# LeeBY68/Hier-SLAM

Measured on AMD Instinct MI355X. Metric: fwd+bwd renders/sec @1200x680, 500k Gaussians, 4-level tree; grad max-abs-err vs ref, higher is better.
Workload: dtype f32; 1 GPU; semantic fwd+bwd render, 1200x680, P=500000 slam Gaussians, K=26 semantic channels, dense upstream grads on colour/semantic/depth/median/opacity; P=500000, visible=480888, num_rendered=1136056, width=1200, height=680, K=26, parallelism=single GPU, keyframes_per_rank=1

## Files before the change

### hier-slam_amd/csrc/hsr_api.hip

```cpp
#include <stdarg.h>

#include <chrono>
#include <time.h>
#include <stdio.h>
#include <stdlib.h>
#include <string.h>

#include <mutex>
#include <type_traits>
#include <vector>

#include "../../include/hsr_rasterizer.h"
#include "hsr_tile_common.h"

namespace {

thread_local char g_err[512] = "";

template <typename T>
inline void take(char*& p, T*& out, size_t count)
{
    uintptr_t a = (reinterpret_cast<uintptr_t>(p) + 255) & ~(uintptr_t)255;
    out = reinterpret_cast<T*>(a);
    p = reinterpret_cast<char*>(out + count);
// ... 134 lines not shown
    if (d < 0 || d >= HSR_MAX_DEVICES) {
        hsr_set_error("device index %d out of range", d);
        return HSR_ERR_INVALID_ARGUMENT;
    }
    g_pc = &g_counters_by_device[d];
    if (!g_pinned) {
        HSR_HIP_CHECK(hipHostMalloc(reinterpret_cast<void**>(&g_pinned), 64, hipHostMallocPortable | hipHostMallocMapped));
        g_pinned[0] = g_pinned[1] = g_pinned[2] = 0;
        HSR_HIP_CHECK(hipHostGetDevicePointer(reinterpret_cast<void**>(&g_pinned_dev), g_pinned, 0));
    }
    return HSR_OK;
}
int read_counter_begin(const uint32_t* dev, hipStream_t stream)
{
    int rc;
    if ((rc = counter_buffer()) != HSR_OK) return rc;
    if (!g_counter_event) HSR_HIP_CHECK(hipEventCreateWithFlags(&g_counter_event, hipEventDisableTiming));
    HSR_HIP_CHECK(hipMemcpyAsync(g_pinned, dev, sizeof(uint32_t), hipMemcpyDeviceToHost, stream));
    HSR_HIP_CHECK(hipMemcpyAsync(g_pinned + 2, dev + 1, sizeof(uint32_t), hipMemcpyDeviceToHost, stream));
    HSR_HIP_CHECK(hipEventRecord(g_counter_event, stream));
    return HSR_OK;
}
thread_local double g_host_wait_ms = 0.0;
thread_local int g_last_per_tile = 0;
int read_counter_end(uint32_t* host_out)
{
    const auto t0 = std::chrono::steady_clock::now();
    HSR_HIP_CHECK(hipEventSynchronize(g_counter_event));
    g_host_wait_ms += std::chrono::duration<double, std::milli>(std::chrono::steady_clock::now() - t0).count();
    *host_out = g_pinned[0];
    return HSR_OK;
}
int poll_counter(uint32_t seq, hipStream_t stream, uint32_t* host_out, volatile uint32_t* slot = nullptr)
{
    const auto t0 = std::chrono::steady_clock::now();
    if (slot) {
        unsigned spins = 0;
        uint32_t cur;
        while ((cur = __atomic_load_n(&slot[1], __ATOMIC_ACQUIRE)) != seq) {
            if (cur != 0 && (int32_t)(cur - seq) > 0) {
                hsr_set_error("non-blocking forward: this call's num_rendered was overwritten — more than %d non-blocking forwards were "
                              "started on the device before it was resolved (resolve or drop earlier ones first)", HSR_ASYNC_SLOTS - 1);
                return HSR_ERR_INVALID_ARGUMENT;
            }
            if ((++spins & 0xFFFu) == 0) {
                const double el = std::chrono::duration<double>(std::chrono::steady_clock::now() - t0).count();
                if (el > 10.0) {
// ... 169 lines not shown
            seq = ++g_counter_seq;
            if (seq == 0) seq = ++g_counter_seq;
            slot_dev = g_pinned_dev;
        }
        StageTimer tm(HSR_STAGE_FWD_DUPLICATE, stream);
        hsr_launch_bin_count(plan, P, radii, tiles_x, tiles_y, g, bin_scratch, im.ranges, stream, slot_dev, seq);
    } else {
        StageTimer tm(HSR_STAGE_FWD_SCAN, stream);
        hsr_launch_scan_block_sums(P, g, stream);
    }
    HSR_LAUNCH_CHECK(in.debug, stream);

    if (!binned && (rc = read_counter_begin(g.counters, stream)) != HSR_OK) return rc;

    RenderFwdArgs ra;
    ra.W = W; ra.H = H; ra.K = in.semantic ? in.K : 0; ra.semantic = in.semantic;
    ra.ranges = im.ranges; ra.point_list = nullptr; ra.masks = nullptr; ra.means2D = g.means2D; ra.conic_opacity = g.conic_opacity;
    ra.depths = g.depths; ra.colors = in.colors_precomp ? in.colors_precomp : g.rgb; ra.semantics = in.semantics;
    ra.rec = g.rec;
    ra.final_T = im.final_T; ra.n_contrib = im.n_contrib; ra.median_pos = im.median_pos;
    ra.out_color = in.out_color; ra.out_semantic = in.out_semantic; ra.out_depth = in.out_depth;
    ra.out_median_depth = in.out_median; ra.out_opacity = in.out_opacity; ra.out_mask = in.out_mask;
    ra.bin = BinDevRef{nullptr, nullptr, 0};
    if (!in.semantic && !in.out_mask) {
        hsr_set_error("out_mask is NULL");
        return HSR_ERR_INVALID_ARGUMENT;
    }

    bool speculated = false;
    if (will_speculate) {
        const BinDevRef ref{static_cast<char*>(binning->ptr), reinterpret_cast<const uint32_t*>(g.counters), binning->capacity};
        BinState none{nullptr, nullptr, nullptr, nullptr, nullptr};
        {
            StageTimer tm(HSR_STAGE_FWD_DUPLICATE, stream);
            hsr_launch_bin_emit(plan, P, radii, tiles_x, tiles_y, g, bin_scratch, im.ranges, nullptr, stream, &ref);
        }
        {
            StageTimer tm(HSR_STAGE_FWD_SORT, stream);
            hsr_launch_tile_sort(none, T, P, im.ranges, stream, &ref, g_last_per_tile);
        }
        ra.bin = ref;
        {
            StageTimer tm(HSR_STAGE_FWD_RENDER, stream);
            hsr_launch_render_forward(ra, stream);
        }
        HSR_HIP_CHECK(hipGetLastError());
        speculated = true;
    }
    if (go_async) {
        ticket->seq = seq;
        ticket->device = slot_device;
        ticket->slot = slot_host;
        ticket->binning_base = static_cast<char*>(binning->ptr);
        ticket->binning_capacity = binning->capacity;
        ticket->prefiltered = in.prefiltered;
        return HSR_PENDING;
    }

    uint32_t R32 = 0;
    if ((rc = binned ? poll_counter(seq, stream, &R32) : read_counter_end(&R32)) != HSR_OK) return rc;
    if (R32 > 0x7fffffffu) {
        hsr_set_error("num_rendered %u overflows int", R32);
        return HSR_ERR_INVALID_ARGUMENT;
    }
    const int R = (int)R32;
    if (in.prefiltered && __atomic_load_n(&g_pinned[2], __ATOMIC_RELAXED) != 0) {
        hsr_set_error("Point is filtered although prefiltered is set. This shouldn't happen!");
        return HSR_ERR_INVALID_ARGUMENT;
    }
    if (speculated) {
        BinState chk;
        const BinDevRef ref{static_cast<char*>(binning->ptr), nullptr, binning->capacity};
        g_last_per_tile = R / (T > 0 ? T : 1);
        if (hsr_bin_resolve(ref, R32, &chk)) return R;
        hsr_launch_bin_count(plan, P, radii, tiles_x, tiles_y, g, bin_scratch, im.ranges, stream, g_pinned_dev, seq);
        ra.bin = BinDevRef{nullptr, nullptr, 0};
    }

    char* bptr;
    if ((rc = acquire(binning, hsr_required_binning_bytes(R), "binning", &bptr)) != HSR_OK) return rc;
    BinState b;
    hsr_carve_bin(bptr, R, &b);

    if (binned) {
        StageTimer tm(HSR_STAGE_FWD_DUPLICATE, stream);
        hsr_launch_bin_emit(plan, P, radii, tiles_x, tiles_y, g, bin_scratch, im.ranges, b.keys, stream);
    }
    if (binned) {
        HSR_LAUNCH_CHECK(in.debug, stream);
        StageTimer tm(HSR_STAGE_FWD_SORT, stream);
        if (R > 0) hsr_launch_tile_sort(b, T, P, im.ranges, stream, nullptr, R / (T > 0 ? T : 1));
    } else {
        const bool emit_sorted = hsr_sort_emit_into_sorted_buffers(end_bit);
        uint64_t* emit_k = emit_sorted ? b.keys : b.keys_unsorted;
        uint32_t* emit_v = emit_sorted ? b.vals : b.vals_unsorted;
        {
            StageTimer tm(HSR_STAGE_FWD_DUPLICATE, stream);
            BinState be = b;
            be.keys_unsorted = emit_k;
            be.vals_unsorted = emit_v;
            hsr_launch_duplicate(P, radii, tiles_x, tiles_y, g, be, im.ranges, stream);
        }
        HSR_LAUNCH_CHECK(in.debug, stream);
        StageTimer tm(HSR_STAGE_FWD_SORT, stream);
        if ((rc = hsr_launch_sort_pairs(b, R, end_bit, T, im.ranges, stream)) != HSR_OK) return rc;
    }
    HSR_LAUNCH_CHECK(in.debug, stream);

    ra.point_list = b.vals;
    ra.masks = b.vals_unsorted;
    {
        StageTimer tm(HSR_STAGE_FWD_RENDER, stream);
        hsr_launch_render_forward(ra, stream);
    }
// ... 480 lines not shown
```

### hier-slam_amd/csrc/hsr_common.h

```cpp
#pragma once
#include <hip/hip_runtime.h>
#include <stddef.h>
#include <stdint.h>

#define HSR_TILE_X 16
#define HSR_TILE_Y 16
#define HSR_TILE_PIX 256
#define HSR_NUM_CHANNELS 3

struct GeomState {
    float* depths;
    float2* means2D;
    float4* conic_opacity;
    float* cov3D;
    float* rgb;
    uint8_t* clamped;
    uint32_t* tiles_touched;
    uint32_t* point_offsets;
    int* radii;
    uint32_t* block_sums;
    uint32_t* counters;
    float4* rec;
};
struct ImgState {
// ... 70 lines not shown
    const float* projmatrix;
    const float* cam_pos;
    float tan_fovx, tan_fovy, focal_x, focal_y;
    int* radii;
    int prefiltered;
    int tiles_x, tiles_y;
};

int hsr_launch_mark_visible(int P, const float* means3D, const float* view, const float* proj, uint8_t* present,
                            hipStream_t stream);
int hsr_launch_preprocess(const PreprocessArgs& a, GeomState& g, hipStream_t stream);
int hsr_launch_scan_block_sums(int P, GeomState& g, hipStream_t stream);
int hsr_launch_duplicate(int P, const int* radii, int tiles_x, int tiles_y, GeomState& g, BinState& b, uint2* ranges,
                         hipStream_t stream);
int hsr_launch_sort_pairs(BinState& b, int R, int end_bit, int T, uint2* ranges, hipStream_t stream);
struct HsrBinPlan { int nblk, per_block; };
bool hsr_bin_plan(int P, int T, size_t scratch_words, HsrBinPlan* plan);
int hsr_launch_bin_count(const HsrBinPlan& plan, int P, const int* radii, int tiles_x, int tiles_y, GeomState& g, uint32_t* scratch,
                         uint2* ranges, hipStream_t stream, uint32_t* host_counter = nullptr, uint32_t host_seq = 0);
int hsr_launch_bin_emit(const HsrBinPlan& plan, int P, const int* radii, int tiles_x, int tiles_y, GeomState& g, const uint32_t* scratch,
                        uint2* ranges, uint64_t* comp, hipStream_t stream, const BinDevRef* ref = nullptr);
int hsr_launch_tile_sort(BinState& b, int T, int P, const uint2* ranges, hipStream_t stream, const BinDevRef* ref = nullptr,
                         int avg_per_tile_hint = 0);
int hsr_sort_tile_passes(int end_bit);
bool hsr_sort_emit_into_sorted_buffers(int end_bit);
int hsr_launch_tile_ranges(int R, int T, const uint64_t* keys, uint2* ranges, hipStream_t stream);
int hsr_launch_tile_ranges_only(int R, const uint64_t* keys, uint2* ranges, hipStream_t stream);

struct RenderFwdArgs {
    int W, H, K, semantic;
    const uint2* ranges;
    const uint32_t* point_list;
    uint32_t* masks;
    const float2* means2D;
    const float4* conic_opacity;
    const float* depths;
    const float* colors;
    const float4* rec;
    const float* semantics;
    float* final_T;
    uint32_t* n_contrib;
    uint32_t* median_pos;
    float* out_color;
    float* out_semantic;
    float* out_depth;
    float* out_median_depth;
    float* out_opacity;
    float* out_mask;
    BinDevRef bin;
};
int hsr_launch_render_forward(const RenderFwdArgs& a, hipStream_t stream);

struct RenderBwdArgs {
    int W, H, K, semantic, P;
    const float* bg;
    const uint2* ranges;
    const uint32_t* point_list;
    const uint32_t* masks;
    const float2* means2D;
    const float4* conic_opacity;
    const float* depths;
    const float* colors;
    const float4* rec;
    const float* final_T;
    const uint32_t* n_contrib;
    const uint32_t* median_pos;
    const float* dL_dpix;
    const float* dL_dpix_sem;
    const float* dL_dpix_depth;
    const float* dL_dpix_median;
    const float* dL_dpix_opacity;
    float* dL_dmean2D;
// ... 59 lines not shown
```

### hier-slam_amd/csrc/hsr_render_fwd.hip

```cpp

#include "hsr_tile_common.h"

#ifdef HSR_TRACE
__device__ unsigned long long g_hsr_trace_fwd[16384 * 8];
extern "C" int hsr_debug_read_trace_fwd(unsigned long long* host, int n)
{
    return (int)hipMemcpyFromSymbol(host, HIP_SYMBOL(g_hsr_trace_fwd), sizeof(unsigned long long) * (size_t)n);
}
#define TRF_NOW() clock64()
#define TRF_ADD(acc, t0) (acc) += (unsigned long long)(clock64() - (t0))
#else
#define TRF_NOW() 0ll
#define TRF_ADD(acc, t0) ((void)0)
#endif

namespace {

template <int W>
__device__ __forceinline__ void quad_fma_words(float (&s)[16], const float (&x)[4], float w)
{
    static_assert(W >= 1 && W <= 4, "1..4 words = 4..16 channels per block");
    if constexpr (W == 4) {
        asm("s_nop 1\n\t"
            "v_fmac_f32_dpp %0, %16, %20 quad_perm:[0,0,0,0] row_mask:0xf bank_mask:0xf\n\t"
// ... 33 lines not shown
    } else if constexpr (W == 2) {
        asm("s_nop 1\n\t"
            "v_fmac_f32_dpp %0, %8, %10 quad_perm:[0,0,0,0] row_mask:0xf bank_mask:0xf\n\t"
            "v_fmac_f32_dpp %1, %8, %10 quad_perm:[1,1,1,1] row_mask:0xf bank_mask:0xf\n\t"
            "v_fmac_f32_dpp %2, %8, %10 quad_perm:[2,2,2,2] row_mask:0xf bank_mask:0xf\n\t"
            "v_fmac_f32_dpp %3, %8, %10 quad_perm:[3,3,3,3] row_mask:0xf bank_mask:0xf\n\t"
            "v_fmac_f32_dpp %4, %9, %10 quad_perm:[0,0,0,0] row_mask:0xf bank_mask:0xf\n\t"
            "v_fmac_f32_dpp %5, %9, %10 quad_perm:[1,1,1,1] row_mask:0xf bank_mask:0xf\n\t"
            "v_fmac_f32_dpp %6, %9, %10 quad_perm:[2,2,2,2] row_mask:0xf bank_mask:0xf\n\t"
            "v_fmac_f32_dpp %7, %9, %10 quad_perm:[3,3,3,3] row_mask:0xf bank_mask:0xf"
            : "+v"(s[0]), "+v"(s[1]), "+v"(s[2]), "+v"(s[3]), "+v"(s[4]), "+v"(s[5]), "+v"(s[6]), "+v"(s[7])
            : "v"(x[0]), "v"(x[1]), "v"(w));
    } else {
        asm("s_nop 1\n\t"
            "v_fmac_f32_dpp %0, %4, %5 quad_perm:[0,0,0,0] row_mask:0xf bank_mask:0xf\n\t"
            "v_fmac_f32_dpp %1, %4, %5 quad_perm:[1,1,1,1] row_mask:0xf bank_mask:0xf\n\t"
            "v_fmac_f32_dpp %2, %4, %5 quad_perm:[2,2,2,2] row_mask:0xf bank_mask:0xf\n\t"
            "v_fmac_f32_dpp %3, %4, %5 quad_perm:[3,3,3,3] row_mask:0xf bank_mask:0xf"
            : "+v"(s[0]), "+v"(s[1]), "+v"(s[2]), "+v"(s[3])
            : "v"(x[0]), "v"(w));
    }
}

template <int KC, bool BASE, bool MASK, bool ALIGNED, bool PF = false>
__global__ void __launch_bounds__(256, KC <= 26 ? (KC == 16 ? 5 : 4) : (PF ? (KC <= 48 ? 4 : (KC <= 80 ? 3 : 2)) : 1)) render_fwd_kernel(RenderFwdArgs a, int c0)
{
    constexpr int BATCH = KC <= 32 ? (KC > 26 ? 200 : 240)
                                   : (KC <= 48 ? 152 : ((KC <= 64 || KC == 74) ? 144 : (KC <= 80 ? 136 : (KC <= 112 ? 144 : 128))));
    static_assert(KC <= 32 || PF, "batch sizes beyond 32 channels assume the touched rows (PF)");
    constexpr int RW = (KC + 2 + 3) & ~3;
    constexpr bool QS = PF && KC > 0;
    constexpr int NGF = QS ? RW / 16 : 0;
    constexpr int REM = QS ? (RW % 16) / 4 : 0;
    __shared__ float4 s_rec[BATCH * 2];
    __shared__ float4 s_row[BATCH * (RW / 4)];
    __shared__ uint8_t s_sublist[16 * HSR_SUB_LSTRIDE];
    __shared__ uint8_t s_subcnt[4][16];
    __shared__ int s_wdone[4];

    const int tile = hsr_block_tile(blockIdx.x, ((a.W + HSR_TILE_X - 1) / HSR_TILE_X) * ((a.H + HSR_TILE_Y - 1) / HSR_TILE_Y));
    if (tile >= ((a.W + HSR_TILE_X - 1) / HSR_TILE_X) * ((a.H + HSR_TILE_Y - 1) / HSR_TILE_Y)) return;
    const int t = threadIdx.x, wv = t >> 6;
    if (a.bin.base) {
        BinState bs;
        if (!hsr_bin_resolve(a.bin, *a.bin.R_dev, &bs)) {
            hsr_poison_tile(a, tile, t, BASE, c0, KC);
            return;
        }
        a.point_list = bs.vals;
        a.masks = bs.vals_unsorted;
    }
    const TileGeom tg = tile_geom_sub(tile, a.W, a.H, t);
    const bool inside = tg.inside;
    const size_t N = (size_t)a.W * a.H;
    float pfx = tg.pfx, pfy = tg.pfy;
    asm volatile("" : "+v"(pfx), "+v"(pfy));
    const float tile_x0 = (float)(tg.tx * HSR_TILE_X), tile_y0 = (float)(tg.ty * HSR_TILE_Y);

    unsigned long long tr_bar = 0, tr_stage = 0, tr_blend = 0, tr_iters = 0, tr_pub = 0;
    (void)tr_pub;
    const long long tr_t0 = TRF_NOW();
    long long tr_t1 = tr_t0;
    (void)tr_bar; (void)tr_stage; (void)tr_blend; (void)tr_iters; (void)tr_t0; (void)tr_t1;
    const uint2 range = a.ranges[tile];
    const int n = (int)(range.y - range.x);

    float T = 1.0f;
    uint32_t last_contributor = 0;
    float C0 = 0, C1 = 0, C2 = 0, Dd = 0, Mm = 0;
    uint32_t median_at = 0;
    float median_D = 15.0f;
    float S[KC > 0 ? KC : 1];
#pragma unroll
// ... 31 lines not shown
            if (KC > 0 && PF) {
                const float* row = a.semantics + id * (size_t)a.K + c0;
                const int last = min(KC, a.K - c0) - 1;
#pragma unroll
                for (int c = 0; c < NPF; c++) pf_t[c] = row[min(16 * c, last)];
            } else if (KC > 0) {
                if (ALIGNED) {
                    const float2* row = reinterpret_cast<const float2*>(a.semantics + id * (size_t)KC);
#pragma unroll
                    for (int q = 0; q < KC / 2; q++) {
                        const float2 v = row[q];
                        p_sem[PF ? 0 : 2 * q] = v.x;
                        p_sem[PF ? 0 : 2 * q + 1] = v.y;
                    }
                } else {
                    const float* row = a.semantics + id * (size_t)a.K + c0;
#pragma unroll
                    for (int c = 0; c < KC; c++) p_sem[PF ? 0 : c] = (c0 + c < a.K) ? row[c] : 0.f;
                }
            }
        }
    };
    if (n > 0) {
        const int id0 = fetch_id(0);
        id_next = fetch_id(BATCH);
        load_record(id0);
    }
    auto resolve_median = [&](int start) {
        if (BASE && median_at > (uint32_t)start) {
            const int j = (int)median_at - 1 - start;
            constexpr int c = KC + 1;
            constexpr int pos = (QS && c / 16 < NGF) ? (16 * (c / 16) + 4 * (c % 4) + (c % 16) / 4) : c;
            median_D = reinterpret_cast<const float*>(s_row)[j * RW + pos];
        }
    };


    for (int start = 0; start < n; start += BATCH) {
        const bool wave_done = __ballot(!done) == 0ull;
        if ((t & 63) == 0) s_wdone[wv] = wave_done;
        const long long tb0 = TRF_NOW();
        (void)tb0;
        __syncthreads();
        TRF_ADD(tr_bar, tb0);
        if (start == 0) tr_t1 = TRF_NOW();
        const long long ts0 = TRF_NOW();
        (void)ts0;
        if (s_wdone[0] & s_wdone[1] & s_wdone[2] & s_wdone[3]) break;
// ... 227 lines not shown
        }
        if (KC > 0) {
#pragma unroll
            for (int c = 0; c < KC; c++)
                if (c0 + c < a.K) a.out_semantic[(size_t)(c0 + c) * N + pix_id] = S[c];
        }
    }
#ifdef HSR_TRACE
    if ((t & 63) == 0) {
        const int wid = tile * 4 + wv;
        if (wid < 16384) {
            unsigned long long* o = g_hsr_trace_fwd + (size_t)wid * 8;
            o[0] = (unsigned long long)(clock64() - tr_t0);
            o[1] = (unsigned long long)(tr_t1 - tr_t0);
            o[2] = tr_bar; o[3] = tr_stage; o[4] = tr_blend;
            o[5] = (unsigned long long)(clock64() - tr_t2);
            o[6] = tr_iters;
            o[7] = tr_pub;
        }
    }
#endif
}

}

int hsr_launch_render_forward(const RenderFwdArgs& a, hipStream_t stream)
{
    const dim3 grid(hsr_tile_grid(((a.W + HSR_TILE_X - 1) / HSR_TILE_X) * ((a.H + HSR_TILE_Y - 1) / HSR_TILE_Y))), block(256);
    if (!a.semantic) {
        render_fwd_kernel<0, true, true, false><<<grid, block, 0, stream>>>(a, 0);
        return HSR_OK;
    }
    if (a.K >= 27 && a.K <= 128 && a.K != 74 && a.K != 102) {
        if (a.K <= 32) render_fwd_kernel<32, true, false, false, true><<<grid, block, 0, stream>>>(a, 0);
        else if (a.K <= 48) render_fwd_kernel<48, true, false, false, true><<<grid, block, 0, stream>>>(a, 0);
        else if (a.K <= 64) render_fwd_kernel<64, true, false, false, true><<<grid, block, 0, stream>>>(a, 0);
        else if (a.K <= 80) render_fwd_kernel<80, true, false, false, true><<<grid, block, 0, stream>>>(a, 0);
        else if (a.K <= 96) render_fwd_kernel<96, true, false, false, true><<<grid, block, 0, stream>>>(a, 0);
        else if (a.K <= 112) render_fwd_kernel<112, true, false, false, true><<<grid, block, 0, stream>>>(a, 0);
        else render_fwd_kernel<128, true, false, false, true><<<grid, block, 0, stream>>>(a, 0);
        return HSR_OK;
    }
    switch (a.K) {
    case 0: render_fwd_kernel<0, true, false, false><<<grid, block, 0, stream>>>(a, 0); return HSR_OK;
    case 16: render_fwd_kernel<16, true, false, true><<<grid, block, 0, stream>>>(a, 0); return HSR_OK;
    case 26: render_fwd_kernel<26, true, false, true><<<grid, block, 0, stream>>>(a, 0); return HSR_OK;
    case 74: render_fwd_kernel<74, true, false, true, true><<<grid, block, 0, stream>>>(a, 0); return HSR_OK;
    case 102: render_fwd_kernel<102, true, false, true, true><<<grid, block, 0, stream>>>(a, 0); return HSR_OK;
    default:
        render_fwd_kernel<32, true, false, false><<<grid, block, 0, stream>>>(a, 0);
        for (int c0 = 32; c0 < a.K; c0 += 32) render_fwd_kernel<32, false, false, false><<<grid, block, 0, stream>>>(a, c0);
        return HSR_OK;
    }
}
```

### hier-slam_amd/csrc/hsr_sort.hip

```cpp
#include "hsr_common.h"

namespace {

constexpr int SORT_THREADS = 256;
constexpr int SORT_ITEMS = 16;
constexpr int SORT_TILE = SORT_THREADS * SORT_ITEMS;
static_assert(SORT_TILE == HSR_SORT_TILE, "hsr_common.h sizes the histogram scratch");

__global__ void __launch_bounds__(SORT_THREADS) sort_hist_kernel(const uint64_t* __restrict__ keys, int n, int shift,
                                                                 uint32_t mask, int nblocks, uint32_t* __restrict__ hist)
{
    __shared__ uint32_t h[256];
    h[threadIdx.x] = 0;
    __syncthreads();
    const int base = blockIdx.x * SORT_TILE;
#pragma unroll 4
    for (int i = 0; i < SORT_ITEMS; i++) {
        const int j = base + i * SORT_THREADS + threadIdx.x;
        if (j < n) atomicAdd(&h[(uint32_t)(keys[j] >> shift) & mask], 1u);
    }
    __syncthreads();
    hist[(size_t)threadIdx.x * nblocks + blockIdx.x] = h[threadIdx.x];
}

// ... 86 lines not shown
        wcnt[0][threadIdx.x] = g;
        wcnt[1][threadIdx.x] = g + c0;
        wcnt[2][threadIdx.x] = g + c0 + c1;
        wcnt[3][threadIdx.x] = g + c0 + c1 + c2;
    }
    __syncthreads();
#pragma unroll
    for (int r = 0; r < SORT_ITEMS; r++) {
        const int j = base + r * 64 + lane;
        if (j < n) {
            const uint32_t d = (uint32_t)(key[r] >> shift) & mask;
            const uint32_t pos = wcnt[w][d] + rank[r];
            kout[pos] = key[r];
            vout[pos] = val[r];
        }
    }
}

}

uint32_t hsr_sort_hist_entries(int R) { return hsr_sort_hist_entries_inline((uint32_t)(R > 0 ? R : 0)); }


constexpr int TS_MAX = 2048;

__device__ __forceinline__ void ts_block_radix(uint64_t* ka, uint32_t* va, uint64_t* kb, uint32_t* vb, int r0, int n,
                                               uint32_t* hist , uint32_t (*wcnt)[256], int gid_passes)
{
    const int t = threadIdx.x, lane = t & 63, w = t >> 6;
    const uint64_t lt = (1ull << lane) - 1ull;
    const int npass = gid_passes + 4;
    for (int pass = 0; pass < npass; pass++) {
        const bool on_gid = pass < gid_passes;
        const int shift = 8 * (on_gid ? pass : pass - gid_passes);
        hist[t] = 0;
#pragma unroll
        for (int i = 0; i < 4; i++) wcnt[i][t] = 0;
        __syncthreads();
        for (int i = t; i < n; i += 256)
            atomicAdd(&hist[((on_gid ? va[r0 + i] : (uint32_t)ka[r0 + i]) >> shift) & 255u], 1u);
        __syncthreads();
        {
            const uint32_t v = hist[t];
            uint32_t inc = v;
#pragma unroll
            for (int o = 1; o < 64; o <<= 1) {
                const uint32_t x = __shfl_up(inc, o);
                if (lane >= o) inc += x;
            }
            __shared__ uint32_t wt[4];
            if (lane == 63) wt[w] = inc;
            __syncthreads();
            uint32_t off = 0;
#pragma unroll
            for (int i = 0; i < 4; i++) off += i < w ? wt[i] : 0u;
            hist[t] = off + inc - v;
        }
        __syncthreads();
        for (int c = 0; c < n; c += 256) {
            const int i = c + t;
            const bool valid = i < n;
            const uint64_t k = valid ? ka[r0 + i] : 0ull;
            const uint32_t v = valid ? va[r0 + i] : 0u;
            const uint32_t d = ((on_gid ? v : (uint32_t)k) >> shift) & 255u;
            uint64_t m = __ballot(valid);
#pragma unroll
            for (int b = 0; b < 8; b++) {
                const bool bit = (d >> b) & 1u;
                const uint64_t bal = __ballot(bit);
                m &= bit ? bal : ~bal;
            }
            const uint32_t before = __popcll(m & lt);
            if (valid && before == 0) wcnt[w][d] = (uint32_t)__popcll(m);
            __syncthreads();
            if (valid) {
                uint32_t pos = hist[d] + before;
#pragma unroll
                for (int i2 = 0; i2 < 4; i2++) pos += i2 < w ? wcnt[i2][d] : 0u;
                kb[r0 + pos] = k;
                vb[r0 + pos] = v;
            }
            __syncthreads();
            hist[t] += wcnt[0][t] + wcnt[1][t] + wcnt[2][t] + wcnt[3][t];
#pragma unroll
            for (int i2 = 0; i2 < 4; i2++) wcnt[i2][t] = 0;
            __syncthreads();
        }
        uint64_t* tk = ka; ka = kb; kb = tk;
        uint32_t* tv = va; va = vb; vb = tv;
        __threadfence_block();
    }
    if (npass & 1) {
        __syncthreads();
        for (int i = t; i < n; i += 256) {
            kb[r0 + i] = ka[r0 + i];
            vb[r0 + i] = va[r0 + i];
        }
    }
}

constexpr int TP_MAX = 1024;
constexpr int TQ_MAX = 2048;

template <int E, int NT>
__device__ __forceinline__ void net_bitonic(uint64_t (&x)[E], int tid, ulonglong2* buf)
{
    constexpr int N = NT * E;
#pragma unroll
    for (int k = 2; k <= N; k <<= 1) {
#pragma unroll
        for (int j = k >> 1; j > 0; j >>= 1) {
            if (j < E) {
#pragma unroll
                for (int r = 0; r < E; r++) {
                    if ((r & j) == 0) {
                        const bool up = k < E ? ((r & k) == 0) : (((E * tid) & k) == 0);
                        const uint64_t a = x[r], b = x[r + j];
                        const bool sw = (a > b) == up;
                        x[r] = sw ? b : a;
                        x[r + j] = sw ? a : b;
                    }
                }
            } else {
                const int m = j / E;
                const bool cross = m >= 64;
#pragma unroll
                for (int q = 0; q < E / 2; q++) buf[q * NT + tid] = make_ulonglong2(x[2 * q], x[2 * q + 1]);
                if (cross) {
                    __syncthreads();
                } else {
                    __builtin_amdgcn_fence(__ATOMIC_RELEASE, "wavefront");
                    __builtin_amdgcn_wave_barrier();
                    __builtin_amdgcn_fence(__ATOMIC_ACQUIRE, "wavefront");
                }
                const bool keep_min = ((tid & m) == 0) == (((E * tid) & k) == 0);
#pragma unroll
                for (int q = 0; q < E / 2; q++) {
                    const ulonglong2 y = buf[q * NT + (tid ^ m)];
                    const uint64_t a0 = x[2 * q], a1 = x[2 * q + 1];
                    x[2 * q] = keep_min ? (a0 < y.x ? a0 : y.x) : (a0 > y.x ? a0 : y.x);
                    x[2 * q + 1] = keep_min ? (a1 < y.y ? a1 : y.y) : (a1 > y.y ? a1 : y.y);
                }
                if (cross) {
                    __syncthreads();
                } else {
                    __builtin_amdgcn_fence(__ATOMIC_RELEASE, "wavefront");
                    __builtin_amdgcn_wave_barrier();
                    __builtin_amdgcn_fence(__ATOMIC_ACQUIRE, "wavefront");
                }
            }
        }
    }
}

__device__ __forceinline__ void block_sort_tile(int tile, const uint2* __restrict__ ranges, uint64_t* __restrict__ keys,
                                                uint32_t* __restrict__ vals, uint64_t* __restrict__ keys_alt,
                                                uint32_t* __restrict__ vals_alt, int gid_passes, int composite_in, uint64_t* comp,
                                                uint32_t* hist, uint32_t (*wcnt)[256])
{
    const uint2 rg = ranges[tile];
    const int r0 = (int)rg.x, n = (int)(rg.y - rg.x);
    const int t = threadIdx.x;
    const uint64_t my_tile_hi = (uint64_t)tile << 32;
    if (n <= 0) return;
    if (n == 1 || n > TS_MAX) {
        if (composite_in) {
            for (int i = t; i < n; i += 256) {
                const uint64_t c = keys[r0 + i];
                keys[r0 + i] = my_tile_hi | (c >> 32);
                vals[r0 + i] = (uint32_t)c;
            }
            __syncthreads();
        }
        if (n == 1) return;
    }
    if (n > TS_MAX) {
// ... 149 lines not shown
    uint32_t* totals = b.hist + (size_t)256 * nblocks;
    uint64_t* ka = (passes & 1) ? b.keys_unsorted : b.keys;
    uint32_t* va = (passes & 1) ? b.vals_unsorted : b.vals;
    uint64_t* kb = (passes & 1) ? b.keys : b.keys_unsorted;
    uint32_t* vb = (passes & 1) ? b.vals : b.vals_unsorted;
    const int bits_per_pass = passes ? (tile_bits + passes - 1) / passes : 0;
    for (int p = 0; p < passes; p++) {
        const int shift = 32 + bits_per_pass * p;
        const int bits = min(bits_per_pass, end_bit - shift);
        const uint32_t mask = (1u << bits) - 1u;
        sort_hist_kernel<<<nblocks, SORT_THREADS, 0, stream>>>(ka, R, shift, mask, nblocks, b.hist);
        sort_rowscan_kernel<<<256, 64, 0, stream>>>(b.hist, nblocks, totals);
        sort_scatter_kernel<<<nblocks, SORT_THREADS, 0, stream>>>(ka, va, kb, vb, R, shift, mask, nblocks, b.hist, totals);
        uint64_t* tk = ka; ka = kb; kb = tk;
        uint32_t* tv = va; va = vb; vb = tv;
    }
    hsr_launch_tile_ranges_only(R, b.keys, ranges, stream);
    tile_sort_kernel<<<T, 256, 0, stream>>>(ranges, b.keys, b.vals, b.keys_unsorted, b.vals_unsorted, 0, 0, BinDevRef{nullptr, nullptr, 0});
    return HSR_OK;
}

int hsr_launch_tile_sort(BinState& b, int T, int P, const uint2* ranges, hipStream_t stream, const BinDevRef* ref, int avg_per_tile_hint)
{
    int bits = 0;
    while (bits < 32 && (1ull << bits) < (unsigned long long)(P > 1 ? P : 1)) bits++;
    const BinDevRef r = ref ? *ref : BinDevRef{nullptr, nullptr, 0};
    const bool many_big = avg_per_tile_hint > 800;
    tile_sort_pair_kernel<<<(T + 1) / 2, 256, 0, stream>>>(T, ranges, b.keys, b.vals, b.keys_unsorted, b.vals_unsorted, (bits + 7) / 8,
                                                           many_big ? 0 : 1, r);
    if (many_big)
        tile_sort_kernel<<<T, 256, 0, stream>>>(ranges, b.keys, b.vals, b.keys_unsorted, b.vals_unsorted, (bits + 7) / 8, 2, r);
    return HSR_OK;
}
```

Baseline: 1742 renders/s.

## Fold per-tile sort into the forward render kernel prologue

Removes the separate tile-sort kernel launch in both the speculative and binned forward paths. Instead, each render block sorts its own tile's composite keys in LDS (bitonic for up to 2048 entries, block radix beyond that) before rendering, and takes the first sorted ids straight from LDS. This saves a kernel launch plus a global round trip of keys and ids. In exchange the render kernel gets a larger LDS footprint, which may lower occupancy, and the sort now runs with the render kernel's launch bounds and per-tile load imbalance.

```diff
diff --git a/hier-slam_amd/csrc/hsr_api.hip b/hier-slam_amd/csrc/hsr_api.hip
--- a/hier-slam_amd/csrc/hsr_api.hip
+++ b/hier-slam_amd/csrc/hsr_api.hip
@@ -180,7 +180,6 @@
     return HSR_OK;
 }
 thread_local double g_host_wait_ms = 0.0;
-thread_local int g_last_per_tile = 0;
 int read_counter_end(uint32_t* host_out)
 {
     const auto t0 = std::chrono::steady_clock::now();
@@ -396,6 +395,7 @@
     ra.out_color = in.out_color; ra.out_semantic = in.out_semantic; ra.out_depth = in.out_depth;
     ra.out_median_depth = in.out_median; ra.out_opacity = in.out_opacity; ra.out_mask = in.out_mask;
     ra.bin = BinDevRef{nullptr, nullptr, 0};
+    ra.sort_fold = 0; ra.sort_gid_passes = 0; ra.sort_keys = nullptr; ra.sort_keys_alt = nullptr; ra.sort_vals = nullptr;
     if (!in.semantic && !in.out_mask) {
         hsr_set_error("out_mask is NULL");
         return HSR_ERR_INVALID_ARGUMENT;
@@ -404,15 +404,12 @@
     bool speculated = false;
     if (will_speculate) {
         const BinDevRef ref{static_cast<char*>(binning->ptr), reinterpret_cast<const uint32_t*>(g.counters), binning->capacity};
-        BinState none{nullptr, nullptr, nullptr, nullptr, nullptr};
         {
             StageTimer tm(HSR_STAGE_FWD_DUPLICATE, stream);
             hsr_launch_bin_emit(plan, P, radii, tiles_x, tiles_y, g, bin_scratch, im.ranges, nullptr, stream, &ref);
         }
-        {
-            StageTimer tm(HSR_STAGE_FWD_SORT, stream);
-            hsr_launch_tile_sort(none, T, P, im.ranges, stream, &ref, g_last_per_tile);
-        }
+        ra.sort_fold = 1;
+        ra.sort_gid_passes = hsr_sort_gid_passes(P);
         ra.bin = ref;
         {
             StageTimer tm(HSR_STAGE_FWD_RENDER, stream);
@@ -445,11 +442,11 @@
     if (speculated) {
         BinState chk;
         const BinDevRef ref{static_cast<char*>(binning->ptr), nullptr, binning->capacity};
-        g_last_per_tile = R / (T > 0 ? T : 1);
         if (hsr_bin_resolve(ref, R32, &chk)) return R;
         hsr_launch_bin_count(plan, P, radii, tiles_x, tiles_y, g, bin_scratch, im.ranges, stream, g_pinned_dev, seq);
         ra.bin = BinDevRef{nullptr, nullptr, 0};
     }
+    ra.sort_fold = 0;
 
     char* bptr;
     if ((rc = acquire(binning, hsr_required_binning_bytes(R), "binning", &bptr)) != HSR_OK) return rc;
@@ -462,8 +459,14 @@
     }
     if (binned) {
         HSR_LAUNCH_CHECK(in.debug, stream);
-        StageTimer tm(HSR_STAGE_FWD_SORT, stream);
-        if (R > 0) hsr_launch_tile_sort(b, T, P, im.ranges, stream, nullptr, R / (T > 0 ? T : 1));
+        if (R > 0 && !in.debug) {
+            ra.sort_fold = 1;
+            ra.sort_gid_passes = hsr_sort_gid_passes(P);
+            ra.sort_keys = b.keys; ra.sort_keys_alt = b.keys_unsorted; ra.sort_vals = b.vals;
+        } else {
+            StageTimer tm(HSR_STAGE_FWD_SORT, stream);
+            if (R > 0) hsr_launch_tile_sort(b, T, P, im.ranges, stream, nullptr, R / (T > 0 ? T : 1));
+        }
     } else {
         const bool emit_sorted = hsr_sort_emit_into_sorted_buffers(end_bit);
         uint64_t* emit_k = emit_sorted ? b.keys : b.keys_unsorted;
diff --git a/hier-slam_amd/csrc/hsr_common.h b/hier-slam_amd/csrc/hsr_common.h
--- a/hier-slam_amd/csrc/hsr_common.h
+++ b/hier-slam_amd/csrc/hsr_common.h
@@ -116,6 +116,12 @@
                         uint2* ranges, uint64_t* comp, hipStream_t stream, const BinDevRef* ref = nullptr);
 int hsr_launch_tile_sort(BinState& b, int T, int P, const uint2* ranges, hipStream_t stream, const BinDevRef* ref = nullptr,
                          int avg_per_tile_hint = 0);
+inline int hsr_sort_gid_passes(int P)
+{
+    int bits = 0;
+    while (bits < 32 && (1ull << bits) < (unsigned long long)(P > 1 ? P : 1)) bits++;
+    return (bits + 7) / 8;
+}
 int hsr_sort_tile_passes(int end_bit);
 bool hsr_sort_emit_into_sorted_buffers(int end_bit);
 int hsr_launch_tile_ranges(int R, int T, const uint64_t* keys, uint2* ranges, hipStream_t stream);
@@ -142,6 +148,9 @@
     float* out_opacity;
     float* out_mask;
     BinDevRef bin;
+    int sort_fold, sort_gid_passes;
+    uint64_t *sort_keys, *sort_keys_alt;
+    uint32_t* sort_vals;
 };
 int hsr_launch_render_forward(const RenderFwdArgs& a, hipStream_t stream);
 
diff --git a/hier-slam_amd/csrc/hsr_render_fwd.hip b/hier-slam_amd/csrc/hsr_render_fwd.hip
--- a/hier-slam_amd/csrc/hsr_render_fwd.hip
+++ b/hier-slam_amd/csrc/hsr_render_fwd.hip
@@ -1,5 +1,6 @@
 
 #include "hsr_tile_common.h"
+#include "hsr_tile_sort.h"
 
 #ifdef HSR_TRACE
 __device__ unsigned long long g_hsr_trace_fwd[16384 * 8];
@@ -79,7 +80,7 @@
     }
 }
 
-template <int KC, bool BASE, bool MASK, bool ALIGNED, bool PF = false>
+template <int KC, bool BASE, bool MASK, bool ALIGNED, bool PF = false, bool SORT = false>
 __global__ void __launch_bounds__(256, KC <= 26 ? (KC == 16 ? 5 : 4) : (PF ? (KC <= 48 ? 4 : (KC <= 80 ? 3 : 2)) : 1)) render_fwd_kernel(RenderFwdArgs a, int c0)
 {
     constexpr int BATCH = KC <= 32 ? (KC > 26 ? 200 : 240)
@@ -89,8 +90,11 @@
     constexpr bool QS = PF && KC > 0;
     constexpr int NGF = QS ? RW / 16 : 0;
     constexpr int REM = QS ? (RW % 16) / 4 : 0;
-    __shared__ float4 s_rec[BATCH * 2];
-    __shared__ float4 s_row[BATCH * (RW / 4)];
+    constexpr int STAGE_BYTES = (BATCH * 2 + BATCH * (RW / 4)) * 16;
+    constexpr int RAW_BYTES = (SORT && STAGE_BYTES < HSR_FOLD_LDS_BYTES) ? HSR_FOLD_LDS_BYTES : STAGE_BYTES;
+    __shared__ __attribute__((aligned(16))) unsigned char s_raw[RAW_BYTES];
+    float4* const s_rec = reinterpret_cast<float4*>(s_raw);
+    float4* const s_row = s_rec + BATCH * 2;
     __shared__ uint8_t s_sublist[16 * HSR_SUB_LSTRIDE];
     __shared__ uint8_t s_subcnt[4][16];
     __shared__ int s_wdone[4];
@@ -106,6 +110,9 @@
         }
         a.point_list = bs.vals;
         a.masks = bs.vals_unsorted;
+        if (SORT) {
+            a.sort_keys = bs.keys; a.sort_vals = bs.vals; a.sort_keys_alt = bs.keys_unsorted;
+        }
     }
     const TileGeom tg = tile_geom_sub(tile, a.W, a.H, t);
     const bool inside = tg.inside;
@@ -183,8 +190,15 @@
         }
     };
     if (n > 0) {
-        const int id0 = fetch_id(0);
-        id_next = fetch_id(BATCH);
+        int id0;
+        if (SORT && fold_sort(tile, (int)range.x, n, t, a.sort_keys, a.sort_vals, a.sort_keys_alt, a.masks, a.sort_gid_passes, s_raw)) {
+            const uint32_t* ids = reinterpret_cast<const uint32_t*>(s_raw + HSR_FOLD_XBUF_BYTES);
+            id0 = (int)ids[min(t, n - 1)];
+            id_next = (int)ids[min(BATCH + t, n - 1)];
+        } else {
+            id0 = fetch_id(0);
+            id_next = fetch_id(BATCH);
+        }
         load_record(id0);
     }
     auto resolve_median = [&](int start) {
@@ -458,34 +472,46 @@
 #endif
 }
 
+template <int KC, bool BASE, bool MASK, bool ALIGNED, bool PF = false>
+void launch_fwd(const RenderFwdArgs& a, int c0, dim3 grid, hipStream_t stream)
+{
+    if constexpr (BASE) {
+        if (a.sort_fold && c0 == 0) {
+            render_fwd_kernel<KC, BASE, MASK, ALIGNED, PF, true><<<grid, dim3(256), 0, stream>>>(a, c0);
+            return;
+        }
+    }
+    render_fwd_kernel<KC, BASE, MASK, ALIGNED, PF, false><<<grid, dim3(256), 0, stream>>>(a, c0);
+}
+
 }
 
 int hsr_launch_render_forward(const RenderFwdArgs& a, hipStream_t stream)
 {
-    const dim3 grid(hsr_tile_grid(((a.W + HSR_TILE_X - 1) / HSR_TILE_X) * ((a.H + HSR_TILE_Y - 1) / HSR_TILE_Y))), block(256);
+    const dim3 grid(hsr_tile_grid(((a.W + HSR_TILE_X - 1) / HSR_TILE_X) * ((a.H + HSR_TILE_Y - 1) / HSR_TILE_Y)));
     if (!a.semantic) {
-        render_fwd_kernel<0, true, true, false><<<grid, block, 0, stream>>>(a, 0);
+        launch_fwd<0, true, true, false>(a, 0, grid, stream);
         return HSR_OK;
     }
     if (a.K >= 27 && a.K <= 128 && a.K != 74 && a.K != 102) {
-        if (a.K <= 32) render_fwd_kernel<32, true, false, false, true><<<grid, block, 0, stream>>>(a, 0);
-        else if (a.K <= 48) render_fwd_kernel<48, true, false, false, true><<<grid, block, 0, stream>>>(a, 0);
-        else if (a.K <= 64) render_fwd_kernel<64, true, false, false, true><<<grid, block, 0, stream>>>(a, 0);
-        else if (a.K <= 80) render_fwd_kernel<80, true, false, false, true><<<grid, block, 0, stream>>>(a, 0);
-        else if (a.K <= 96) render_fwd_kernel<96, true, false, false, true><<<grid, block, 0, stream>>>(a, 0);
-        else if (a.K <= 112) render_fwd_kernel<112, true, false, false, true><<<grid, block, 0, stream>>>(a, 0);
-        else render_fwd_kernel<128, true, false, false, true><<<grid, block, 0, stream>>>(a, 0);
+        if (a.K <= 32) launch_fwd<32, true, false, false, true>(a, 0, grid, stream);
+        else if (a.K <= 48) launch_fwd<48, true, false, false, true>(a, 0, grid, stream);
+        else if (a.K <= 64) launch_fwd<64, true, false, false, true>(a, 0, grid, stream);
+        else if (a.K <= 80) launch_fwd<80, true, false, false, true>(a, 0, grid, stream);
+        else if (a.K <= 96) launch_fwd<96, true, false, false, true>(a, 0, grid, stream);
+        else if (a.K <= 112) launch_fwd<112, true, false, false, true>(a, 0, grid, stream);
+        else launch_fwd<128, true, false, false, true>(a, 0, grid, stream);
         return HSR_OK;
     }
     switch (a.K) {
-    case 0: render_fwd_kernel<0, true, false, false><<<grid, block, 0, stream>>>(a, 0); return HSR_OK;
-    case 16: render_fwd_kernel<16, true, false, true><<<grid, block, 0, stream>>>(a, 0); return HSR_OK;
-    case 26: render_fwd_kernel<26, true, false, true><<<grid, block, 0, stream>>>(a, 0); return HSR_OK;
-    case 74: render_fwd_kernel<74, true, false, true, true><<<grid, block, 0, stream>>>(a, 0); return HSR_OK;
-    case 102: render_fwd_kernel<102, true, false, true, true><<<grid, block, 0, stream>>>(a, 0); return HSR_OK;
+    case 0: launch_fwd<0, true, false, false>(a, 0, grid, stream); return HSR_OK;
+    case 16: launch_fwd<16, true, false, true>(a, 0, grid, stream); return HSR_OK;
+    case 26: launch_fwd<26, true, false, true>(a, 0, grid, stream); return HSR_OK;
+    case 74: launch_fwd<74, true, false, true, true>(a, 0, grid, stream); return HSR_OK;
+    case 102: launch_fwd<102, true, false, true, true>(a, 0, grid, stream); return HSR_OK;
     default:
-        render_fwd_kernel<32, true, false, false><<<grid, block, 0, stream>>>(a, 0);
-        for (int c0 = 32; c0 < a.K; c0 += 32) render_fwd_kernel<32, false, false, false><<<grid, block, 0, stream>>>(a, c0);
+        launch_fwd<32, true, false, false>(a, 0, grid, stream);
+        for (int c0 = 32; c0 < a.K; c0 += 32) launch_fwd<32, false, false, false>(a, c0, grid, stream);
         return HSR_OK;
     }
 }
diff --git a/hier-slam_amd/csrc/hsr_sort.hip b/hier-slam_amd/csrc/hsr_sort.hip
--- a/hier-slam_amd/csrc/hsr_sort.hip
+++ b/hier-slam_amd/csrc/hsr_sort.hip
@@ -1,4 +1,5 @@
 #include "hsr_common.h"
+#include "hsr_tile_sort.h"
 
 namespace {
 
@@ -132,136 +133,9 @@
 uint32_t hsr_sort_hist_entries(int R) { return hsr_sort_hist_entries_inline((uint32_t)(R > 0 ? R : 0)); }
 
 
-constexpr int TS_MAX = 2048;
-
-__device__ __forceinline__ void ts_block_radix(uint64_t* ka, uint32_t* va, uint64_t* kb, uint32_t* vb, int r0, int n,
-                                               uint32_t* hist , uint32_t (*wcnt)[256], int gid_passes)
-{
-    const int t = threadIdx.x, lane = t & 63, w = t >> 6;
-    const uint64_t lt = (1ull << lane) - 1ull;
-    const int npass = gid_passes + 4;
-    for (int pass = 0; pass < npass; pass++) {
-        const bool on_gid = pass < gid_passes;
-        const int shift = 8 * (on_gid ? pass : pass - gid_passes);
-        hist[t] = 0;
-#pragma unroll
-        for (int i = 0; i < 4; i++) wcnt[i][t] = 0;
-        __syncthreads();
-        for (int i = t; i < n; i += 256)
-            atomicAdd(&hist[((on_gid ? va[r0 + i] : (uint32_t)ka[r0 + i]) >> shift) & 255u], 1u);
-        __syncthreads();
-        {
-            const uint32_t v = hist[t];
-            uint32_t inc = v;
-#pragma unroll
-            for (int o = 1; o < 64; o <<= 1) {
-                const uint32_t x = __shfl_up(inc, o);
-                if (lane >= o) inc += x;
-            }
-            __shared__ uint32_t wt[4];
-            if (lane == 63) wt[w] = inc;
-            __syncthreads();
-            uint32_t off = 0;
-#pragma unroll
-            for (int i = 0; i < 4; i++) off += i < w ? wt[i] : 0u;
-            hist[t] = off + inc - v;
-        }
-        __syncthreads();
-        for (int c = 0; c < n; c += 256) {
-            const int i = c + t;
-            const bool valid = i < n;
-            const uint64_t k = valid ? ka[r0 + i] : 0ull;
-            const uint32_t v = valid ? va[r0 + i] : 0u;
-            const uint32_t d = ((on_gid ? v : (uint32_t)k) >> shift) & 255u;
-            uint64_t m = __ballot(valid);
-#pragma unroll
-            for (int b = 0; b < 8; b++) {
-                const bool bit = (d >> b) & 1u;
-                const uint64_t bal = __ballot(bit);
-                m &= bit ? bal : ~bal;
-            }
-            const uint32_t before = __popcll(m & lt);
-            if (valid && before == 0) wcnt[w][d] = (uint32_t)__popcll(m);
-            __syncthreads();
-            if (valid) {
-                uint32_t pos = hist[d] + before;
-#pragma unroll
-                for (int i2 = 0; i2 < 4; i2++) pos += i2 < w ? wcnt[i2][d] : 0u;
-                kb[r0 + pos] = k;
-                vb[r0 + pos] = v;
-            }
-            __syncthreads();
-            hist[t] += wcnt[0][t] + wcnt[1][t] + wcnt[2][t] + wcnt[3][t];
-#pragma unroll
-            for (int i2 = 0; i2 < 4; i2++) wcnt[i2][t] = 0;
-            __syncthreads();
-        }
-        uint64_t* tk = ka; ka = kb; kb = tk;
-        uint32_t* tv = va; va = vb; vb = tv;
-        __threadfence_block();
-    }
-    if (npass & 1) {
-        __syncthreads();
-        for (int i = t; i < n; i += 256) {
-            kb[r0 + i] = ka[r0 + i];
-            vb[r0 + i] = va[r0 + i];
-        }
-    }
-}
 
 constexpr int TP_MAX = 1024;
 constexpr int TQ_MAX = 2048;
-
-template <int E, int NT>
-__device__ __forceinline__ void net_bitonic(uint64_t (&x)[E], int tid, ulonglong2* buf)
-{
-    constexpr int N = NT * E;
-#pragma unroll
-    for (int k = 2; k <= N; k <<= 1) {
-#pragma unroll
-        for (int j = k >> 1; j > 0; j >>= 1) {
-            if (j < E) {
-#pragma unroll
-                for (int r = 0; r < E; r++) {
-                    if ((r & j) == 0) {
-                        const bool up = k < E ? ((r & k) == 0) : (((E * tid) & k) == 0);
-                        const uint64_t a = x[r], b = x[r + j];
-                        const bool sw = (a > b) == up;
-                        x[r] = sw ? b : a;
-                        x[r + j] = sw ? a : b;
-                    }
-                }
-            } else {
-                const int m = j / E;
-                const bool cross = m >= 64;
-#pragma unroll
-                for (int q = 0; q < E / 2; q++) buf[q * NT + tid] = make_ulonglong2(x[2 * q], x[2 * q + 1]);
-                if (cross) {
-                    __syncthreads();
-                } else {
-                    __builtin_amdgcn_fence(__ATOMIC_RELEASE, "wavefront");
-                    __builtin_amdgcn_wave_barrier();
-                    __builtin_amdgcn_fence(__ATOMIC_ACQUIRE, "wavefront");
-                }
-                const bool keep_min = ((tid & m) == 0) == (((E * tid) & k) == 0);
-#pragma unroll
-                for (int q = 0; q < E / 2; q++) {
-                    const ulonglong2 y = buf[q * NT + (tid ^ m)];
-                    const uint64_t a0 = x[2 * q], a1 = x[2 * q + 1];
-                    x[2 * q] = keep_min ? (a0 < y.x ? a0 : y.x) : (a0 > y.x ? a0 : y.x);
-                    x[2 * q + 1] = keep_min ? (a1 < y.y ? a1 : y.y) : (a1 > y.y ? a1 : y.y);
-                }
-                if (cross) {
-                    __syncthreads();
-                } else {
-                    __builtin_amdgcn_fence(__ATOMIC_RELEASE, "wavefront");
-                    __builtin_amdgcn_wave_barrier();
-                    __builtin_amdgcn_fence(__ATOMIC_ACQUIRE, "wavefront");
-                }
-            }
-        }
-    }
-}
 
 __device__ __forceinline__ void block_sort_tile(int tile, const uint2* __restrict__ ranges, uint64_t* __restrict__ keys,
                                                 uint32_t* __restrict__ vals, uint64_t* __restrict__ keys_alt,
@@ -457,13 +331,11 @@
 
 int hsr_launch_tile_sort(BinState& b, int T, int P, const uint2* ranges, hipStream_t stream, const BinDevRef* ref, int avg_per_tile_hint)
 {
-    int bits = 0;
-    while (bits < 32 && (1ull << bits) < (unsigned long long)(P > 1 ? P : 1)) bits++;
     const BinDevRef r = ref ? *ref : BinDevRef{nullptr, nullptr, 0};
     const bool many_big = avg_per_tile_hint > 800;
-    tile_sort_pair_kernel<<<(T + 1) / 2, 256, 0, stream>>>(T, ranges, b.keys, b.vals, b.keys_unsorted, b.vals_unsorted, (bits + 7) / 8,
+    tile_sort_pair_kernel<<<(T + 1) / 2, 256, 0, stream>>>(T, ranges, b.keys, b.vals, b.keys_unsorted, b.vals_unsorted, hsr_sort_gid_passes(P),
                                                            many_big ? 0 : 1, r);
     if (many_big)
-        tile_sort_kernel<<<T, 256, 0, stream>>>(ranges, b.keys, b.vals, b.keys_unsorted, b.vals_unsorted, (bits + 7) / 8, 2, r);
+        tile_sort_kernel<<<T, 256, 0, stream>>>(ranges, b.keys, b.vals, b.keys_unsorted, b.vals_unsorted, hsr_sort_gid_passes(P), 2, r);
     return HSR_OK;
 }
diff --git a/hier-slam_amd/csrc/hsr_tile_sort.h b/hier-slam_amd/csrc/hsr_tile_sort.h
--- /dev/null
+++ b/hier-slam_amd/csrc/hsr_tile_sort.h
@@ -0,0 +1,177 @@
+#pragma once
+#include "hsr_common.h"
+
+constexpr int TS_MAX = 2048;
+
+__device__ __forceinline__ void ts_block_radix(uint64_t* ka, uint32_t* va, uint64_t* kb, uint32_t* vb, int r0, int n,
+                                               uint32_t* hist , uint32_t (*wcnt)[256], int gid_passes)
+{
+    const int t = threadIdx.x, lane = t & 63, w = t >> 6;
+    const uint64_t lt = (1ull << lane) - 1ull;
+    const int npass = gid_passes + 4;
+    for (int pass = 0; pass < npass; pass++) {
+        const bool on_gid = pass < gid_passes;
+        const int shift = 8 * (on_gid ? pass : pass - gid_passes);
+        hist[t] = 0;
+#pragma unroll
+        for (int i = 0; i < 4; i++) wcnt[i][t] = 0;
+        __syncthreads();
+        for (int i = t; i < n; i += 256)
+            atomicAdd(&hist[((on_gid ? va[r0 + i] : (uint32_t)ka[r0 + i]) >> shift) & 255u], 1u);
+        __syncthreads();
+        {
+            const uint32_t v = hist[t];
+            uint32_t inc = v;
+#pragma unroll
+            for (int o = 1; o < 64; o <<= 1) {
+                const uint32_t x = __shfl_up(inc, o);
+                if (lane >= o) inc += x;
+            }
+            __shared__ uint32_t wt[4];
+            if (lane == 63) wt[w] = inc;
+            __syncthreads();
+            uint32_t off = 0;
+#pragma unroll
+            for (int i = 0; i < 4; i++) off += i < w ? wt[i] : 0u;
+            hist[t] = off + inc - v;
+        }
+        __syncthreads();
+        for (int c = 0; c < n; c += 256) {
+            const int i = c + t;
+            const bool valid = i < n;
+            const uint64_t k = valid ? ka[r0 + i] : 0ull;
+            const uint32_t v = valid ? va[r0 + i] : 0u;
+            const uint32_t d = ((on_gid ? v : (uint32_t)k) >> shift) & 255u;
+            uint64_t m = __ballot(valid);
+#pragma unroll
+            for (int b = 0; b < 8; b++) {
+                const bool bit = (d >> b) & 1u;
+                const uint64_t bal = __ballot(bit);
+                m &= bit ? bal : ~bal;
+            }
+            const uint32_t before = __popcll(m & lt);
+            if (valid && before == 0) wcnt[w][d] = (uint32_t)__popcll(m);
+            __syncthreads();
+            if (valid) {
+                uint32_t pos = hist[d] + before;
+#pragma unroll
+                for (int i2 = 0; i2 < 4; i2++) pos += i2 < w ? wcnt[i2][d] : 0u;
+                kb[r0 + pos] = k;
+                vb[r0 + pos] = v;
+            }
+            __syncthreads();
+            hist[t] += wcnt[0][t] + wcnt[1][t] + wcnt[2][t] + wcnt[3][t];
+#pragma unroll
+            for (int i2 = 0; i2 < 4; i2++) wcnt[i2][t] = 0;
+            __syncthreads();
+        }
+        uint64_t* tk = ka; ka = kb; kb = tk;
+        uint32_t* tv = va; va = vb; vb = tv;
+        __threadfence_block();
+    }
+    if (npass & 1) {
+        __syncthreads();
+        for (int i = t; i < n; i += 256) {
+            kb[r0 + i] = ka[r0 + i];
+            vb[r0 + i] = va[r0 + i];
+        }
+    }
+}
+
+template <int E, int NT>
+__device__ __forceinline__ void net_bitonic(uint64_t (&x)[E], int tid, ulonglong2* buf)
+{
+    constexpr int N = NT * E;
+#pragma unroll
+    for (int k = 2; k <= N; k <<= 1) {
+#pragma unroll
+        for (int j = k >> 1; j > 0; j >>= 1) {
+            if (j < E) {
+#pragma unroll
+                for (int r = 0; r < E; r++) {
+                    if ((r & j) == 0) {
+                        const bool up = k < E ? ((r & k) == 0) : (((E * tid) & k) == 0);
+                        const uint64_t a = x[r], b = x[r + j];
+                        const bool sw = (a > b) == up;
+                        x[r] = sw ? b : a;
+                        x[r + j] = sw ? a : b;
+                    }
+                }
+            } else {
+                const int m = j / E;
+                const bool cross = m >= 64;
+#pragma unroll
+                for (int q = 0; q < E / 2; q++) buf[q * NT + tid] = make_ulonglong2(x[2 * q], x[2 * q + 1]);
+                if (cross) {
+                    __syncthreads();
+                } else {
+                    __builtin_amdgcn_fence(__ATOMIC_RELEASE, "wavefront");
+                    __builtin_amdgcn_wave_barrier();
+                    __builtin_amdgcn_fence(__ATOMIC_ACQUIRE, "wavefront");
+                }
+                const bool keep_min = ((tid & m) == 0) == (((E * tid) & k) == 0);
+#pragma unroll
+                for (int q = 0; q < E / 2; q++) {
+                    const ulonglong2 y = buf[q * NT + (tid ^ m)];
+                    const uint64_t a0 = x[2 * q], a1 = x[2 * q + 1];
+                    x[2 * q] = keep_min ? (a0 < y.x ? a0 : y.x) : (a0 > y.x ? a0 : y.x);
+                    x[2 * q + 1] = keep_min ? (a1 < y.y ? a1 : y.y) : (a1 > y.y ? a1 : y.y);
+                }
+                if (cross) {
+                    __syncthreads();
+                } else {
+                    __builtin_amdgcn_fence(__ATOMIC_RELEASE, "wavefront");
+                    __builtin_amdgcn_wave_barrier();
+                    __builtin_amdgcn_fence(__ATOMIC_ACQUIRE, "wavefront");
+                }
+            }
+        }
+    }
+}
+
+constexpr int HSR_FOLD_XBUF_BYTES = 4 * 256 * 16;
+constexpr int HSR_FOLD_LDS_BYTES = HSR_FOLD_XBUF_BYTES + TS_MAX * 4;
+template <int E>
+__device__ __forceinline__ void fold_sort_tile(int r0, int n, int t, uint64_t tile_hi, uint64_t* keys, uint32_t* vals, ulonglong2* xbuf,
+                                               uint32_t* ids)
+{
+    uint64_t x[E];
+#pragma unroll
+    for (int r = 0; r < E; r++) {
+        const int e = E * t + r;
+        x[r] = e < n ? keys[r0 + e] : ~0ull;
+    }
+    net_bitonic<E, 256>(x, t, xbuf);
+#pragma unroll
+    for (int r = 0; r < E; r++) {
+        const int e = E * t + r;
+        if (e < n) {
+            keys[r0 + e] = tile_hi | (x[r] >> 32);
+            vals[r0 + e] = (uint32_t)x[r];
+            ids[e] = (uint32_t)x[r];
+        }
+    }
+}
+
+__device__ __forceinline__ bool fold_sort(int tile, int r0, int n, int t, uint64_t* keys, uint32_t* vals, uint64_t* keys_alt,
+                                          uint32_t* vals_alt, int gid_passes, unsigned char* lds)
+{
+    const uint64_t tile_hi = (uint64_t)tile << 32;
+    ulonglong2* xbuf = reinterpret_cast<ulonglong2*>(lds);
+    uint32_t* ids = reinterpret_cast<uint32_t*>(lds + HSR_FOLD_XBUF_BYTES);
+    if (n <= 512) fold_sort_tile<2>(r0, n, t, tile_hi, keys, vals, xbuf, ids);
+    else if (n <= 1024) fold_sort_tile<4>(r0, n, t, tile_hi, keys, vals, xbuf, ids);
+    else if (n <= TS_MAX) fold_sort_tile<8>(r0, n, t, tile_hi, keys, vals, xbuf, ids);
+    else {
+        for (int i = t; i < n; i += 256) {
+            const uint64_t c = keys[r0 + i];
+            keys[r0 + i] = tile_hi | (c >> 32);
+            vals[r0 + i] = (uint32_t)c;
+        }
+        __syncthreads();
+        uint32_t* hist = reinterpret_cast<uint32_t*>(lds);
+        ts_block_radix(keys, vals, keys_alt, vals_alt, r0, n, hist, reinterpret_cast<uint32_t (*)[256]>(hist + 256), gid_passes);
+    }
+    __syncthreads();
+    return n <= TS_MAX;
+}
```

Result: no change. 1757 renders/s (median of 3 runs) (+0.9%).
